# summa-dev/halo2-experiments

Measured on AMD Instinct MI355X. Metric: BN256 G1 MSM throughput, higher is better.
Workload: dtype u32; 1 GPU; standalone BN256 G1 MSM, 2^24 points per GPU (global 2^24 x 1; BASELINE configs[4] microbench, north-star headline size); points_per_gpu=16777216, global_points=16777216, base_set=fixed-base table (registration default from 2^17 points), window_bits=22, windows=12, parallelism=index-range shards x1, all-gather of 96 B partials (RCCL) + host fold, base_set_bytes=12901679104

## Files before the change

### halo2-experiments_amd/_lib.py

```python
from __future__ import annotations

import ctypes
import os
import subprocess

_HERE = os.path.dirname(os.path.abspath(__file__))
CSRC = os.path.join(_HERE, "csrc")
os.environ.setdefault("GPU_MAX_HW_QUEUES", "16")
LIB_PATH = os.environ.get("HALO2_MI355X_LIB") or os.path.join(CSRC, "libhalo2_mi355x.so")
HOSTCHECK_PATH = os.path.join(CSRC, "libhm_hostcheck.so")
HEADER_PATH = os.path.join(os.path.dirname(_HERE), "include", "halo2_mi355x.h")

_u64p = ctypes.POINTER(ctypes.c_uint64)
_vp = ctypes.c_void_p
NO_CHAIN = ctypes.c_size_t(-1).value


class Halo2Mi355xError(RuntimeError):
    def __init__(self, code: int, message: str):
        super().__init__(f"libhalo2_mi355x error {code}: {message}")
        self.code = code


class MsmStats(ctypes.Structure):
# ... 44 lines not shown
                                          ctypes.POINTER(ctypes.c_int)]),
    "hm_register_bases_dev": (ctypes.c_int, [_vp, ctypes.c_size_t, _vp, _u64p]),
    "hm_register_bases_precomp": (ctypes.c_int, [_u64p, ctypes.c_size_t, _u64p]),
    "hm_register_bases_precomp_dev": (ctypes.c_int, [_vp, ctypes.c_size_t, _vp, _u64p]),
    "hm_register_bases_plain": (ctypes.c_int, [_u64p, ctypes.c_size_t, _u64p]),
    "hm_register_bases_plain_dev": (ctypes.c_int, [_vp, ctypes.c_size_t, _vp, _u64p]),
    "hm_get_bases_info": (ctypes.c_int, [ctypes.c_uint64, ctypes.POINTER(BasesInfo)]),
    "hm_msm_bn256_g1_dev": (ctypes.c_int, [ctypes.c_uint64, ctypes.c_size_t, _vp, ctypes.c_size_t, _vp, _u64p]),
    "hm_msm_submit_dev": (ctypes.c_int, [ctypes.c_uint64, ctypes.c_size_t, _vp, ctypes.c_size_t, _vp, _u64p]),
    "hm_msm_wait": (ctypes.c_int, [ctypes.c_uint64, _u64p]),
    "hm_msm_batch_bn256_g1_dev": (ctypes.c_int, [ctypes.c_uint64, ctypes.c_size_t, ctypes.POINTER(ctypes.c_void_p), ctypes.c_size_t,
                                                 ctypes.c_size_t, _vp, _u64p]),
    "hm_msm_batch_bn256_g1_h": (ctypes.c_int, [ctypes.c_uint64, ctypes.c_size_t, ctypes.POINTER(ctypes.c_void_p), ctypes.c_size_t,
                                              ctypes.c_size_t, _u64p]),
    "hm_g1_sum": (ctypes.c_int, [_u64p, ctypes.c_size_t, _u64p]),
    "hm_coeff_to_extended_bn256_fr_dev": (ctypes.c_int, [ctypes.c_void_p, ctypes.c_void_p, ctypes.c_size_t, _u64p, ctypes.c_uint32,
                                                         ctypes.c_uint32, _u64p, ctypes.c_void_p]),
    "hm_coeff_to_coset_bn256_fr_dev": (ctypes.c_int, [_vp, _vp, ctypes.c_size_t, _u64p, ctypes.c_uint32, _u64p, ctypes.c_int, _vp]),
    "hm_coset_to_coeff_bn256_fr_dev": (ctypes.c_int, [_vp, ctypes.c_size_t, _u64p, ctypes.c_uint32, _u64p, _u64p, _vp]),
    "hm_coeff_to_cosets_bn256_fr_dev": (ctypes.c_int, [_vp, _vp, ctypes.c_size_t, _u64p, ctypes.c_uint32, _u64p, ctypes.c_size_t, ctypes.c_int, _vp]),
    "hm_cosets_to_coeff_bn256_fr_dev": (ctypes.c_int, [_vp, ctypes.c_size_t, _u64p, ctypes.c_uint32, _u64p, _u64p, _vp]),
    "hm_msm_set_window": (ctypes.c_int, [ctypes.c_int]),
    "hm_msm_set_phase_timing": (ctypes.c_int, [ctypes.c_int]),
    "hm_set_host_base_cache": (ctypes.c_int, [ctypes.c_int]),
    "hm_set_fixed_base_threshold": (ctypes.c_int, [ctypes.c_uint32]),
    "hm_set_msm_devices": (ctypes.c_int, [ctypes.POINTER(ctypes.c_int), ctypes.c_int]),
    "hm_ntt_bn256_fr": (ctypes.c_int, [_u64p, _u64p, ctypes.c_uint32]),
    "hm_set_host_copies": (ctypes.c_int, [ctypes.c_int]),
    "hm_host_register": (ctypes.c_int, [ctypes.c_void_p, ctypes.c_size_t]),
    "hm_host_unregister": (ctypes.c_int, [ctypes.c_void_p]),
# ... 100 lines not shown
```

### halo2-experiments_amd/csrc/capi.hip

```cpp
#include <hip/hip_runtime.h>

#include <cstdlib>

#include <atomic>
#include <chrono>
#include <string>
#include <map>
#include <random>
#include <stdexcept>
#include <thread>
#include <vector>

#include "hm_internal.h"
#include "host_fr.h"

namespace hm {

namespace {
struct HwQueueDefault {
  HwQueueDefault() { (void)setenv("GPU_MAX_HW_QUEUES", "16", 0); }
} g_hw_queue_default;
}

static thread_local std::string g_last_error;
// ... 33 lines not shown
long g_fault_after = -1;
void hm_fault_point(const char* point) {
  std::lock_guard<std::mutex> lk(g_fault_mu);
  if (g_fault_after < 0 || g_fault_name != point) return;
  if (g_fault_after-- == 0) throw std::runtime_error(std::string("injected fault at ") + point);
}
#endif

void msm_set_window_override(int c);
void msm_set_phase_timing(int mode);

static double now_us() {
  return std::chrono::duration<double, std::micro>(std::chrono::steady_clock::now().time_since_epoch()).count();
}

static void count_msm(DeviceCtx& ctx, size_t n, double device_ms) {
  uint32_t lg = 0;
  while ((n >> (lg + 1)) != 0) ++lg;
  ctx.calls.msm_calls += 1;
  ctx.calls.msm_points += n;
  ctx.calls.msm_by_log[lg & 31] += 1;
  ctx.calls.msm_device_us += device_ms * 1e3;
}

constexpr size_t kParkedBytesMax = (size_t)2 << 30;
static size_t parked_bytes(const DeviceCtx& ctx) {
  size_t t = 0;
  for (const auto& f : ctx.free_bases) t += f.xy_bytes + f.inf_bytes;
  return t;
}
static void free_bases_entry(DeviceCtx& ctx, BasesEntry& b) {
// ... 433 lines not shown
  if (!b) return hm_fail(HM_ERR_NOT_FOUND, "hm_get_bases_info: unknown handle");
  out->n = b->n;
  out->table_windows = b->pc_W;
  out->table_window_bits = b->pc_c;
  out->device_bytes = b->xy_bytes + b->inf_bytes;
  out->devices = 1;
  out->parked_bytes = parked_bytes(*ctx);
  return HM_OK;
} HM_API_CATCH("hm_get_bases_info")

int hm_release_bases(uint64_t handle) try {
  if (is_multi_handle(handle)) return multi_release(handle);
  DeviceCtx* ctx = ctx_for_current_device();
  if (!ctx) return HM_ERR_NO_DEVICE;
  std::lock_guard<std::mutex> lk(ctx->mu);
  for (size_t i = 0; i < ctx->bases.size(); ++i) {
    if (ctx->bases[i].handle == handle) {
      bool in_flight = false;
      for (int k = 1; k < HM_MSM_SLOTS; ++k)
        if (ctx->msm_slots[k].busy && ctx->msm_slots[k].bases_handle == handle) in_flight = true;
      if (in_flight) ctx->zombie_bases.push_back(ctx->bases[i]);
      else free_bases_entry(*ctx, ctx->bases[i]);
      ctx->bases.erase(ctx->bases.begin() + i);
      return HM_OK;
    }
  }
  return hm_fail(HM_ERR_NOT_FOUND, "hm_release_bases: unknown handle");
} HM_API_CATCH("hm_release_bases")

int hm_msm_bn256_g1_dev(uint64_t handle, size_t offset, const void* d_scalars, size_t n, void* stream, uint64_t out_xyz[12]) try {
// ... 3 lines not shown
    return multi_msm(handle, offset, d_scalars, false, n, stream, out_xyz, &id);
  }
  DeviceCtx* ctx = ctx_for_current_device();
  if (!ctx) return HM_ERR_NO_DEVICE;
  std::lock_guard<std::mutex> lk(ctx->mu);
  BasesEntry* b = find_bases(*ctx, handle);
  if (!b) return hm_fail(HM_ERR_NOT_FOUND, "hm_msm_bn256_g1_dev: unknown base handle");
  if (offset > b->n || n > b->n - offset) return hm_fail(HM_ERR_BAD_ARG, "hm_msm_bn256_g1_dev: offset + n exceeds the base set");
  int is_id = 0;
  const uint32_t pc = (offset == 0 && n == b->n) ? b->pc_c : 0u;
  const int rc = msm_run(*ctx, (const uint32_t*)d_scalars, b->d_xy + offset * 16, b->d_inf + offset, n, pc, out_xyz, &is_id,
                         (hipStream_t)stream);
  if (rc == HM_OK) count_msm(*ctx, n, ctx->last_msm.t_total_ms);
  return rc;
} HM_API_CATCH("hm_msm_bn256_g1_dev")

static int submit_chain(DeviceCtx* ctx, uint64_t handle, size_t offset, const void* const* d_scalars_list, uint32_t group, size_t n,
                        void* stream, uint64_t* out_ticket, const char* who, bool* all_busy = nullptr, bool use_table = true,
                        size_t live_rows = 0) {
  if (all_busy) *all_busy = false;
  std::lock_guard<std::mutex> lk(ctx->mu);
  BasesEntry* b = find_bases(*ctx, handle);
  if (!b) return hm_fail(HM_ERR_NOT_FOUND, std::string(who) + ": unknown base handle");
  if (offset > b->n || n > b->n - offset) return hm_fail(HM_ERR_BAD_ARG, std::string(who) + ": offset + n exceeds the base set");
  int slot = -1;
  for (int i = 1; i < HM_MSM_SLOTS; ++i)
    if (!ctx->msm_slots[i].busy) { slot = i; break; }
  if (slot < 0) {
    if (all_busy) *all_busy = true;
    return hm_fail(HM_ERR_BAD_ARG, std::string(who) + ": every slot is in flight; hm_msm_wait one first");
// ... 582 lines not shown

int hm_g1_sum(const uint64_t* points_xyz, size_t count, uint64_t out_xyz[12]) try {
  if (!out_xyz || (count && !points_xyz)) return hm_fail(HM_ERR_BAD_ARG, "hm_g1_sum: null argument");
  if (count > (1u << 20)) return hm_fail(HM_ERR_BAD_ARG, "hm_g1_sum: meant for a handful of partial results");
  hm_fault_point("g1_sum");
  int is_id = 0;
  host_sum_points(points_xyz, count, out_xyz, &is_id);
  return HM_OK;
} HM_API_CATCH("hm_g1_sum")

int hm_get_msm_stats(hm_msm_stats* out) try {
  if (!out) return hm_fail(HM_ERR_BAD_ARG, "hm_get_msm_stats: null output");
  DeviceCtx* ctx = ctx_for_current_device();
  if (!ctx) return HM_ERR_NO_DEVICE;
  std::lock_guard<std::mutex> lk(ctx->mu);
  const MsmStats& s = ctx->last_msm;
  out->digits_ms = s.t_digits_ms; out->sort_ms = s.t_sort_ms; out->accumulate_ms = s.t_accum_ms;
  out->reduce_ms = s.t_reduce_ms; out->total_ms = s.t_total_ms; out->accumulate_kernel_ms = s.t_accum_kernel_ms;
  out->pairs = s.pairs; out->tasks = s.tasks; out->window_bits = s.c; out->windows = s.windows;
  return HM_OK;
} HM_API_CATCH("hm_get_msm_stats")

int hm_get_stats(hm_stats* out) try {
  if (!out) return hm_fail(HM_ERR_BAD_ARG, "hm_get_stats: null output");
  DeviceCtx* ctx = ctx_for_current_device();
  if (!ctx) return HM_ERR_NO_DEVICE;
  std::lock_guard<std::mutex> lk(ctx->mu);
  const CallStats& c = ctx->calls;
  std::memset(out, 0, sizeof *out);
  out->msm_calls = c.msm_calls; out->msm_points = c.msm_points;
  out->ntt_calls = c.ntt_calls; out->ntt_elements = c.ntt_elements;
  for (int i = 0; i < 32; ++i) { out->msm_calls_by_log2[i] = c.msm_by_log[i]; out->ntt_calls_by_log2[i] = c.ntt_by_log[i]; }
  out->msm_h2d_us = c.msm_h2d_us; out->msm_device_us = c.msm_device_us; out->msm_host_us = c.msm_host_us;
  out->ntt_h2d_us = c.ntt_h2d_us; out->ntt_device_us = c.ntt_device_us; out->ntt_d2h_us = c.ntt_d2h_us;
  out->h2d_bytes = c.h2d_bytes; out->d2h_bytes = c.d2h_bytes;
  for (int i = 0; i < 8; ++i) { out->vector_calls[i] = c.vector_calls[i]; out->vector_elements[i] = c.vector_elements[i]; }
  out->coset_table_bytes = ctx->coset_table_bytes;
  out->coset_tables = ctx->coset_tables.size();
  out->ntt_table_bytes = ctx->ntt_table_bytes;
  out->ntt_tables = ctx->ntt_tables.size();
  out->host_copies_direct = ctx->xfer.direct.load(std::memory_order_relaxed);
  out->host_copies_staged = ctx->xfer.staged.load(std::memory_order_relaxed);
// ... 739 lines not shown
```

### halo2-experiments_amd/csrc/hm_internal.h

```cpp
#pragma once
#include <hip/hip_runtime.h>
#include <stdint.h>

#include <atomic>
#include <cstring>
#include <exception>
#include <functional>
#include <memory>
#include <mutex>
#include <string>
#include <thread>
#include <utility>
#include <vector>

#include "../../include/halo2_mi355x.h"

namespace hm {

int hm_fail(int code, const std::string& what);

#define HM_HIP_CHECK(expr)                                                                          \
  do {                                                                                              \
    hipError_t _e = (expr);                                                                         \
    if (_e != hipSuccess)                                                                           \
// ... 210 lines not shown
  std::vector<BasesEntry> zombie_bases;
  std::vector<FreeBases> free_bases;
  std::vector<std::unique_ptr<GraphProgram>> graphs;
  hipStream_t batch_streams[HM_MSM_SLOTS - 1] = {};
  hipEvent_t batch_event = nullptr;
  bool batch_streams_ready = false;
  DevBuf batch_io[HM_MSM_SLOTS - 1];
  DevBuf live_io;
  std::mutex live_mu;
  std::mutex batch_h_mu;
  uint64_t next_handle = 1;
  size_t cached_host_n = 0;
  const void* cached_xy = nullptr;
  uint64_t cached_digest[4] = {0, 0, 0, 0};
  MsmStats last_msm;
  CallStats calls;
  bool msm_attr_set = false, ntt_attr_set = false, msm_small_attr_set = false, lookup_attr_set = false;
};

AuxSlot* aux_acquire(DeviceCtx& ctx, hipStream_t stream);
int aux_release(DeviceCtx& ctx, AuxSlot* slot, hipStream_t stream);

DeviceCtx* ctx_for_current_device();

int xfer_h2d(DeviceCtx& ctx, void* d_dst, const void* src, size_t bytes, const char* who);
int xfer_d2h(DeviceCtx& ctx, void* dst, const void* d_src, size_t bytes, const char* who);
int xfer_many(DeviceCtx& ctx, bool up, void* const* dev, void* const* host, const size_t* bytes, size_t count, const char* who);
void xfer_release(DeviceCtx& ctx);
void xfer_prefault(void* p, size_t bytes);
int xfer_set_policy(int mode);
// ... 88 lines not shown
bool msm_phase_timing(bool small_plan);
int msm_slot_prepare(MsmSlot& sl);
int msm_launch_digits(const uint32_t* d_scalars_ext, const uint8_t* d_inf, int32_t* d_digits, size_t n, uint32_t c, uint32_t W,
                      hipStream_t stream);
bool msm_small_applies(size_t n, uint32_t c, bool single_set);
int msm_issue_small(DeviceCtx& ctx, int slot, const uint32_t* const* d_scalars_list, uint32_t group, const uint32_t* d_xy,
                    const uint8_t* d_inf, size_t n, uint32_t c, hipStream_t stream);
int msm_count_live_blocks(DeviceCtx& ctx, const void* const* d_columns, size_t count, const uint8_t* d_inf, size_t n, hipStream_t stream,
                          uint32_t* live_out);
bool msm_group_applies(size_t n, uint32_t precomp_c);
int msm_enqueue_group(DeviceCtx& ctx, int slot, const uint32_t* const* d_scalars_list, uint32_t group, const uint32_t* d_xy,
                      const uint8_t* d_inf, size_t n, hipStream_t stream, size_t live_rows = 0);
int msm_run(DeviceCtx& ctx, const uint32_t* d_scalars_ext, const uint32_t* d_xy, const uint8_t* d_inf, size_t n,
            uint32_t precomp_c, uint64_t out_jac_ext[12], int* out_is_identity, hipStream_t stream);
uint32_t msm_precomp_window(size_t n);
int msm_precompute(uint32_t* d_table, const uint8_t* d_inf, size_t n, uint32_t c, uint32_t W, hipStream_t stream);
void host_sum_points(const uint64_t* pts, size_t count, uint64_t out_jac_ext[12], int* out_is_identity);
int g1_fixed_base_mul_run(DeviceCtx& ctx, const uint32_t* d_scalars_ext, size_t n, const uint64_t base_affine_ext[8],
                          uint32_t* d_out_affine_ext, hipStream_t stream);

}
```

### halo2-experiments_amd/csrc/msm.hip

```cpp
#include <hip/hip_runtime.h>

#include <algorithm>
#include <chrono>
#include <cmath>
#include <cstdlib>

#include "hm_internal.h"
#include "host_fq.h"
#include "msm_dev.h"

namespace hm {


__global__ void msm_init_counters_kernel(uint32_t* __restrict__ bcnt, size_t nbt, uint32_t* __restrict__ br_count,
                                         uint32_t* __restrict__ khist, uint32_t nkeys, uint32_t* __restrict__ big_count) {
  const size_t i0 = (size_t)blockIdx.x * blockDim.x + threadIdx.x, stride = (size_t)gridDim.x * blockDim.x;
  for (size_t i = i0; i < nbt; i += stride) bcnt[i] = 0;
  if (i0 < nkeys) khist[i0] = 0;
  if (i0 < 4) {
    if (br_count) br_count[i0] = 0;
    big_count[i0] = 0;
  }
}

// ... 21 lines not shown

#ifndef HM_TARGET_TASKS
#define HM_TARGET_TASKS 327680
#endif
constexpr uint32_t TARGET_TASKS = HM_TARGET_TASKS;
__device__ __forceinline__ uint32_t effective_task_len(const uint32_t* __restrict__ pairs, uint32_t L_host) {
  if (pairs == nullptr) return L_host;
  const uint32_t by_fill = pairs[0] / TARGET_TASKS;
  const uint32_t L = L_host < by_fill ? L_host : by_fill;
  return L < 16u ? 16u : L;
}

struct MsmGroupScalars {
  const uint32_t* s[HM_MSM_GROUP];
};
__global__ void msm_digits_kernel(MsmGroupScalars list, const uint8_t* __restrict__ inf,
                                  int32_t* __restrict__ digits, size_t n, uint32_t c, uint32_t W, uint32_t n_wide) {
  const size_t i = (size_t)blockIdx.x * blockDim.x + threadIdx.x;
  if (i >= n) return;
  const uint32_t* __restrict__ scalars = list.s[blockIdx.y];
  digits += (size_t)blockIdx.y * W * n;
  const uint4* q = reinterpret_cast<const uint4*>(scalars + i * 8);
  const uint4 lo = q[0], hi = q[1];
  const uint32_t w_in[8] = {lo.x, lo.y, lo.z, lo.w, hi.x, hi.y, hi.z, hi.w};
  Fr k32 = fe_zero<FrParams>();
  k32.l[0] = 32;
  const Fr s = fe_canonical(fe_mul(fe_unpack<FrParams>(w_in), k32));
  uint32_t v[9];
  {
    uint32_t t[8];
    fe_pack(t, s);
#pragma unroll
    for (int k = 0; k < 8; ++k) v[k] = t[k];
    v[8] = 0;
  }
  const bool skip = inf[i] != 0;
  uint32_t carry = 0;
  for (uint32_t w = 0; w < W; ++w) {
    const uint32_t bits = w < n_wide ? c : c - 1;
    const uint32_t mask = (1u << bits) - 1u, half = 1u << (bits - 1);
    uint32_t d = (v[0] & mask) + carry;
    int32_t sd;
    if (d > half) {
      sd = (int32_t)d - (int32_t)(1u << bits);
      carry = 1;
    } else {
      sd = (int32_t)d;
      carry = 0;
    }
    digits[(size_t)w * n + i] = skip ? 0 : (w < n_wide ? sd : 2 * sd);
#pragma unroll
    for (int k = 0; k < 8; ++k) v[k] = __funnelshift_r(v[k], v[k + 1], bits);
  }
}

#ifndef HM_SORT_THREADS
#define HM_SORT_THREADS 1024
#endif
constexpr int SORT_THREADS = HM_SORT_THREADS;

template <class T, class F>
__device__ __forceinline__ void block_for_each_word(const T* __restrict__ base, size_t lo, size_t hi, F f) {
  size_t a = lo;
  while (a < hi && (reinterpret_cast<uintptr_t>(base + a) & (4 * sizeof(T) - 1))) ++a;
  const size_t nvec = (hi - a) / 4;
  if (threadIdx.x < a - lo) f(lo + threadIdx.x, base[lo + threadIdx.x]);
  const size_t tail = a + nvec * 4;
  if (threadIdx.x < hi - tail) f(tail + threadIdx.x, base[tail + threadIdx.x]);
// ... 12 lines not shown
__global__ __launch_bounds__(SORT_THREADS) void msm_part1_hist_kernel(const int32_t* __restrict__ digits,
                                                                      uint32_t* __restrict__ chist, size_t n, size_t chunk,
                                                                      uint32_t fb, uint32_t NC) {
  extern __shared__ uint32_t hist[];
  const uint32_t g = blockIdx.x, w = blockIdx.y, G = gridDim.x;
  for (uint32_t b = threadIdx.x; b < NC; b += SORT_THREADS) hist[b] = 0;
  __syncthreads();
  const size_t lo = (size_t)g * chunk, hi = lo + chunk < n ? lo + chunk : n;
  const int32_t* dw = digits + (size_t)w * n;
  block_for_each_word(dw, lo, hi, [&](size_t, int32_t d) {
    if (d != 0) (void)lds_inc(hist, ((uint32_t)(d < 0 ? -d : d) - 1u) >> fb);
  });
  __syncthreads();
  uint32_t* out = chist + ((size_t)w * G + g) * NC;
  for (uint32_t b = threadIdx.x; b < NC; b += SORT_THREADS) out[b] = hist[b];
}

__global__ __launch_bounds__(64) void msm_part1_scan_kernel(uint32_t* __restrict__ chist, uint32_t* __restrict__ ctot, uint32_t G,
                                                            uint32_t NC, uint32_t W) {
  const uint32_t idx = blockIdx.x;
  if (idx >= W * NC) return;
  const uint32_t w = idx / NC, b = idx - w * NC;
  const uint32_t lane = threadIdx.x;
  const uint32_t per = (G + 63) / 64;
  const uint32_t lo = lane * per, hi = lo + per < G ? lo + per : G;
  uint32_t sum = 0;
  for (uint32_t g = lo; g < hi; ++g) sum += chist[((size_t)w * G + g) * NC + b];
  uint32_t incl = sum;
#pragma unroll
  for (int off = 1; off < 64; off <<= 1) {
// ... 1429 lines not shown
  return v;
}

struct BigRegionPlan {
  uint32_t big = 0;
  uint32_t slice = 0;
  uint32_t capacity = 0;
  uint2* list = nullptr;
  uint32_t* count = nullptr;
  uint32_t* gcursor = nullptr;
};

template <class ITEM>
static int launch_sort(const int32_t* d_digits, uint32_t* d_chist, uint32_t* d_ctot, uint32_t* d_cstart, void* d_tmp,
                       uint32_t* d_bcnt, size_t sn, size_t chunk, uint32_t G, uint32_t SW, uint32_t fb, uint32_t ib, uint32_t cb,
                       uint32_t NC, uint32_t NBP, const BigRegionPlan& br, hipStream_t stream) {
  const size_t lds_fine = (size_t)4 << fb;
  if (cb) {
    const size_t lds_coarse = (size_t)NC * 4;
    hipLaunchKernelGGL(msm_part1_hist_kernel, dim3(G, SW), dim3(SORT_THREADS), lds_coarse, stream, d_digits, d_chist, sn, chunk,
                       fb, NC);
    hipLaunchKernelGGL(msm_part1_scan_kernel, dim3(SW * NC), dim3(64), 0, stream, d_chist, d_ctot, G, NC, SW);
    hipLaunchKernelGGL(msm_part1_starts_kernel, dim3(1), dim3(1024), 0, stream, (const uint32_t*)d_ctot, d_cstart, SW * NC);
    static const bool big_tiles = [] { const char* v = std::getenv("HALO2_MI355X_P1_BIG_TILES"); return !(v && *v == '0'); }();
    static const uint32_t p1_big_from = [] { const char* v = std::getenv("HALO2_MI355X_P1_BIG_FROM"); return (uint32_t)(v && *v ? std::atoi(v) : 512); }();
    if (sizeof(ITEM) == 4 && NC <= 4096 && !sort_v1()) {
      if (NC >= (p1_big_from) && NC <= 2048 && big_tiles) {
        constexpr int TILE = SORT_THREADS * P1_BIG_IPT;
        hipLaunchKernelGGL((msm_part1_scatter_v2_kernel<P1_BIG_IPT>), dim3(G, SW), dim3(SORT_THREADS), ((size_t)3 * NC + 32 + 2 * TILE) * 4, stream,
                           d_digits, (const uint32_t*)d_chist, (const uint32_t*)d_cstart, (uint32_t*)d_tmp, sn, chunk, fb, ib, NC);
      } else {
        constexpr int TILE = SORT_THREADS * P1_IPT_DEFAULT;
        hipLaunchKernelGGL((msm_part1_scatter_v2_kernel<P1_IPT_DEFAULT>), dim3(G, SW), dim3(SORT_THREADS), ((size_t)3 * NC + 32 + 2 * TILE) * 4,
                           stream, d_digits, (const uint32_t*)d_chist, (const uint32_t*)d_cstart, (uint32_t*)d_tmp, sn, chunk, fb, ib, NC);
      }
    } else if (NC >= (p1_big_from) && NC <= 2048 && sizeof(ITEM) == 4 && big_tiles) {
// ... 301 lines not shown
  sl.res_stride = res_stride;
  sl.live_ptr = nullptr;
  sl.phase_timed = msm_phase_timing(false);
  const bool pt = sl.phase_timed;
  sl.T_max = T_max;
  sl.d_win = d_win;
  sl.d_tot = d_tot;
  HM_HIP_CHECK(hipEventRecord(ev[0], stream));

  uint32_t n_wide = W;
  if (single_set) {
    uint32_t wide;
    balanced_windows(W, &wide, &n_wide);
    if (wide != c) return hm_fail(HM_ERR_INTERNAL, "msm: the base set's table was built for another window split");
  }
  {
    MsmGroupScalars list;
    for (uint32_t e = 0; e < (uint32_t)HM_MSM_GROUP; ++e) list.s[e] = d_scalars_list[e < group ? e : 0];
    hipLaunchKernelGGL(msm_digits_kernel, dim3((uint32_t)((n + 255) / 256), group), dim3(256), 0, stream, list, d_inf, d_digits, n, c, W,
                       n_wide);
  }
  HM_HIP_CHECK(hipGetLastError());
  if (pt) HM_HIP_CHECK(hipEventRecord(ev[1], stream));

  {
    {
      const uint32_t blocks = (uint32_t)std::min<size_t>(((size_t)NBT + 255) / 256, 2048);
      hipLaunchKernelGGL(msm_init_counters_kernel, dim3(blocks < 4 ? 4 : blocks), dim3(256), 0, stream, d_bcnt, (size_t)NBT,
                         cb ? br.count : (uint32_t*)nullptr, d_khist, TASK_KEYS, d_big_count);
      HM_HIP_CHECK(hipGetLastError());
    }
    const int rc = wide_items
                       ? launch_sort<uint64_t>(d_digits, d_chist, d_ctot, d_cstart, d_tmp, d_bcnt, sn, chunk, G, SW, fb, ib, cb,
                                               NC, NBP, br, stream)
                       : launch_sort<uint32_t>(d_digits, d_chist, d_ctot, d_cstart, d_tmp, d_bcnt, sn, chunk, G, SW, fb, ib, cb,
                                               NC, NBP, br, stream);
    if (rc != HM_OK) return rc;
  }
  const uint32_t* d_pairs = cb ? (const uint32_t*)(d_cstart + (size_t)SW * NC) : (const uint32_t*)nullptr;
  {
    const uint32_t nblocks = (NBT + SCAN_BLOCK - 1) / SCAN_BLOCK;
    hipLaunchKernelGGL(msm_scan_partial_kernel, dim3(nblocks), dim3(SCAN_THREADS), 0, stream, (const uint32_t*)d_bcnt,
                       d_bsum, NBT, d_pairs, L);
    hipLaunchKernelGGL(msm_scan_blocksums_kernel, dim3(1), dim3(SCAN_THREADS), 0, stream, d_bsum, nblocks, d_tot,
                       (uint32_t)std::min<uint64_t>(T_max, 0xffffffffull));
    hipLaunchKernelGGL(msm_scan_final_kernel, dim3(nblocks), dim3(SCAN_THREADS), 0, stream, (const uint32_t*)d_bcnt,
                       (const uint32_t*)d_bsum, d_boff, d_toff, (const uint32_t*)d_tot, NBT, d_pairs, L,
                       coop_sort ? br.gcursor : (uint32_t*)nullptr);
    HM_HIP_CHECK(hipGetLastError());
  }
  {
// ... 172 lines not shown
  ctx.last_msm.c = sl.c;
  ctx.last_msm.windows = sl.W;
}

int msm_finish(DeviceCtx& ctx, int slot, uint64_t out_jac_ext[12], int* out_is_identity) {
  double host_us = 0;
  const int rc = msm_finish_wait_fold(ctx.msm_slots[slot], out_jac_ext, out_is_identity, &host_us);
  if (rc == HM_OK) msm_finish_record(ctx, slot, host_us);
  else ctx.msm_slots[slot].live_ptr = nullptr;
  return rc;
}

int msm_run(DeviceCtx& ctx, const uint32_t* d_scalars_ext, const uint32_t* d_xy, const uint8_t* d_inf, size_t n,
            uint32_t precomp_c, uint64_t out_jac_ext[12], int* out_is_identity, hipStream_t stream) {
  if (ctx.msm_slots[0].busy) return hm_fail(HM_ERR_BAD_ARG, "msm: slot 0 is held by an un-awaited hm_msm_submit_dev ticket");
  const int rc = msm_enqueue(ctx, 0, d_scalars_ext, d_xy, d_inf, n, precomp_c, stream);
  if (rc != HM_OK) return rc;
  return msm_finish(ctx, 0, out_jac_ext, out_is_identity);
}

int g1_fixed_base_mul_run(DeviceCtx& ctx, const uint32_t* d_scalars_ext, size_t n, const uint64_t base_affine_ext[8],
                          uint32_t* d_out_affine_ext, hipStream_t stream) {
  if (n == 0) return HM_OK;
  AuxSlot* slot = aux_acquire(ctx, stream);
  if (!slot) return HM_ERR_HIP;
  uint32_t* d_table = (uint32_t*)slot->table.ensure((size_t)64 * 15 * PT_WORDS * 4);
  if (!d_table) return hm_fail(HM_ERR_HIP, "fixed-base: table allocation failed");
  G1AffineWords base;
  std::memcpy(base.w, base_affine_ext, 64);
  hipLaunchKernelGGL(g1_fixed_table_kernel, dim3(1), dim3(64), 0, stream, base, d_table);
  HM_HIP_CHECK(hipGetLastError());
  hipLaunchKernelGGL(g1_fixed_base_mul_kernel, dim3((uint32_t)((n + ACC_THREADS - 1) / ACC_THREADS)), dim3(ACC_THREADS), 0,
                     stream, d_scalars_ext, (const uint32_t*)d_table, d_out_affine_ext, n);
// ... 6 lines not shown
```

### halo2-experiments_amd/sharding.py

```python
from __future__ import annotations

import ctypes
import os
from typing import Callable, Optional, Tuple

import numpy as np

from . import _lib
from .arithmetic import _ptr, best_multiexp


def shard_range(n: int, rank: int, world: int) -> Tuple[int, int]:
    if not (0 <= rank < world):
        raise ValueError("rank out of range")
    q, r = divmod(n, world)
    lo = rank * q + min(rank, r)
    return lo, lo + q + (1 if rank < r else 0)


def g1_sum(points: np.ndarray) -> np.ndarray:
    pts = np.ascontiguousarray(points, dtype=np.uint64).reshape(-1, 12)
    out = np.zeros(12, dtype=np.uint64)
    _lib.check(_lib.load().hm_g1_sum(_ptr(pts), pts.shape[0], _ptr(out)))
    return out
# ... 11 lines not shown
    return bool(force_collective)


def _comm_device(group):
    import torch
    import torch.distributed as dist

    return torch.device("cuda", torch.cuda.current_device()) if dist.get_backend(group) == "nccl" else torch.device("cpu")


def sharded_multiexp(local_coeffs, local_bases, group=None,
                     local_msm: Optional[Callable] = None, force_collective: Optional[bool] = None) -> np.ndarray:
    import torch
    import torch.distributed as dist

    partial = (local_msm or best_multiexp)(local_coeffs, local_bases)
    if not _exchanges(group, force_collective):
        return g1_sum(partial.reshape(1, 12))
    world = dist.get_world_size(group)
    dev = _comm_device(group)
    mine = torch.from_numpy(partial.view(np.int64).copy()).to(dev)
    gathered = [torch.empty_like(mine) for _ in range(world)]
    dist.all_gather(gathered, mine, group=group)
    pts = torch.stack(gathered).cpu().numpy().view(np.uint64)
    return g1_sum(pts)


MAX_IN_FLIGHT = 8
_NO_GROUP = object()


def sharded_multiexp_batch(jobs, group=None, streams=None, local_batch: Optional[Callable] = None,
                           force_collective: Optional[bool] = None) -> np.ndarray:
    import torch
    import torch.distributed as dist

    if local_batch is not None:
        partials = np.stack([np.asarray(p, dtype=np.uint64).reshape(12) for p in local_batch(jobs)]) if jobs else np.zeros((0, 12), np.uint64)
    else:
        partials = np.zeros((len(jobs), 12), dtype=np.uint64)
# ... 92 lines not shown
```

### include/halo2_mi355x.h

```cpp
#ifndef HALO2_MI355X_H
#define HALO2_MI355X_H

#include <stddef.h>
#include <stdint.h>

#ifdef __cplusplus
extern "C" {
#endif

#define HM_OK 0
#define HM_ERR_BAD_ARG (-1)
#define HM_ERR_NO_DEVICE (-2)
#define HM_ERR_HIP (-3)
#define HM_ERR_NOT_FOUND (-4)
#define HM_ERR_INTERNAL (-5)
#define HM_ERR_PARTIAL_OUTPUT (-6)


int hm_set_device(int device);
int hm_device_count(void);
int hm_shutdown(void);
const char* hm_last_error(void);
const char* hm_version(void);

// ... 16 lines not shown
typedef struct hm_bases_info {
  uint64_t n;
  uint64_t device_bytes;
  uint64_t parked_bytes;
  uint64_t default_tables_dropped;
  uint32_t table_windows;
  uint32_t table_window_bits;
  uint32_t devices;
  uint32_t sliced;
} hm_bases_info;
int hm_get_bases_info(uint64_t handle, hm_bases_info* out);

int hm_register_bases_dev(const void* d_bases, size_t n, void* stream, uint64_t* out_handle);
int hm_msm_bn256_g1_dev(uint64_t handle, size_t offset, const void* d_scalars, size_t n, void* stream,
                        uint64_t out_xyz[12]);

int hm_msm_submit_dev(uint64_t handle, size_t offset, const void* d_scalars, size_t n, void* stream, uint64_t* out_ticket);
int hm_msm_wait(uint64_t ticket, uint64_t out_xyz[12]);
int hm_msm_batch_bn256_g1_dev(uint64_t handle, size_t offset, const void* const* d_scalars, size_t n, size_t count, void* stream,
                              uint64_t* out_xyz);
int hm_msm_batch_bn256_g1_h(uint64_t handle, size_t offset, const uint64_t* const* scalars, size_t n, size_t count, uint64_t* out_xyz);

int hm_set_msm_devices(const int* devices, int count);

int hm_g1_sum(const uint64_t* points_xyz, size_t count, uint64_t out_xyz[12]);

int hm_set_host_base_cache(int enable);

int hm_device_malloc(size_t bytes, void** d_out);
int hm_device_free(void* d_ptr);
// ... 136 lines not shown
```

### rust/halo2-mi355x-sys/src/lib.rs

```rust
#![allow(non_camel_case_types)]

use std::ffi::CStr;
use std::os::raw::{c_char, c_int, c_long, c_void};

pub const HM_OK: c_int = 0;
pub const HM_ERR_BAD_ARG: c_int = -1;
pub const HM_ERR_NO_DEVICE: c_int = -2;
pub const HM_ERR_HIP: c_int = -3;
pub const HM_ERR_NOT_FOUND: c_int = -4;
pub const HM_ERR_INTERNAL: c_int = -5;
pub const HM_ERR_PARTIAL_OUTPUT: c_int = -6;
pub const HM_GRAPH_COLUMNS_INTERNAL: c_int = 1;
pub const HM_STAT_EVAL_POLYNOMIAL: c_int = 0;
pub const HM_STAT_GRAPH_EVALUATE: c_int = 1;
pub const HM_STAT_KATE_DIVISION: c_int = 2;
pub const HM_STAT_GRAND_PRODUCT: c_int = 3;
pub const HM_STAT_BATCH_INVERT: c_int = 4;
pub const HM_STAT_LINEAR_COMBINATION: c_int = 5;
pub const HM_STAT_LOOKUP_PERMUTE: c_int = 6;

#[repr(C)]
#[derive(Clone, Copy, Debug)]
pub struct HmBasesInfo {
    pub n: u64,
    pub device_bytes: u64,
    pub parked_bytes: u64,
// ... 54 lines not shown
    pub fn hm_last_error() -> *const c_char;
    pub fn hm_version() -> *const c_char;
    pub fn hm_msm_bn256_g1(scalars: *const u64, bases: *const u64, n: usize, out_xy: *mut u64, out_is_identity: *mut c_int) -> c_int;
    pub fn hm_msm_bn256_g1_jacobian(scalars: *const u64, bases: *const u64, n: usize, out_xyz: *mut u64) -> c_int;
    pub fn hm_register_bases(bases: *const u64, n: usize, out_handle: *mut u64) -> c_int;
    pub fn hm_release_bases(handle: u64) -> c_int;
    pub fn hm_msm_bn256_g1_h(handle: u64, offset: usize, scalars: *const u64, n: usize, out_xy: *mut u64, out_is_identity: *mut c_int) -> c_int;
    pub fn hm_register_bases_precomp(bases: *const u64, n: usize, out_handle: *mut u64) -> c_int;
    pub fn hm_register_bases_precomp_dev(d_bases: *const c_void, n: usize, stream: *mut c_void, out_handle: *mut u64) -> c_int;
    pub fn hm_set_fixed_base_threshold(log2_n: u32) -> c_int;
    pub fn hm_register_bases_plain(bases: *const u64, n: usize, out_handle: *mut u64) -> c_int;
    pub fn hm_register_bases_plain_dev(d_bases: *const c_void, n: usize, stream: *mut c_void, out_handle: *mut u64) -> c_int;
    pub fn hm_get_bases_info(handle: u64, out: *mut HmBasesInfo) -> c_int;
    pub fn hm_register_bases_dev(d_bases: *const c_void, n: usize, stream: *mut c_void, out_handle: *mut u64) -> c_int;
    pub fn hm_msm_bn256_g1_dev(handle: u64, offset: usize, d_scalars: *const c_void, n: usize, stream: *mut c_void, out_xyz: *mut u64) -> c_int;
    pub fn hm_msm_submit_dev(handle: u64, offset: usize, d_scalars: *const c_void, n: usize, stream: *mut c_void, out_ticket: *mut u64) -> c_int;
    pub fn hm_msm_wait(ticket: u64, out_xyz: *mut u64) -> c_int;
    pub fn hm_msm_batch_bn256_g1_dev(handle: u64, offset: usize, d_scalars: *const *const c_void, n: usize, count: usize,
        stream: *mut c_void, out_xyz: *mut u64) -> c_int;
    pub fn hm_msm_batch_bn256_g1_h(handle: u64, offset: usize, scalars: *const *const u64, n: usize, count: usize, out_xyz: *mut u64) -> c_int;
    pub fn hm_set_msm_devices(devices: *const c_int, count: c_int) -> c_int;
    pub fn hm_g1_sum(points_xyz: *const u64, count: usize, out_xyz: *mut u64) -> c_int;
    pub fn hm_set_host_base_cache(enable: c_int) -> c_int;
    pub fn hm_device_malloc(bytes: usize, d_out: *mut *mut c_void) -> c_int;
    pub fn hm_device_free(d_ptr: *mut c_void) -> c_int;
    pub fn hm_copy_to_device(d_dst: *mut c_void, src: *const c_void, bytes: usize) -> c_int;
    pub fn hm_copy_to_host(dst: *mut c_void, d_src: *const c_void, bytes: usize) -> c_int;
    pub fn hm_copy_many_to_device(d_dsts: *const *mut c_void, srcs: *const *const c_void, bytes: *const usize, count: usize) -> c_int;
    pub fn hm_copy_many_to_host(dsts: *const *mut c_void, d_srcs: *const *const c_void, bytes: *const usize, count: usize) -> c_int;
    pub fn hm_device_synchronize() -> c_int;
// ... 77 lines not shown
```

Before: 948.4 million points/s.

## Fuse digit extraction with coarse histogram and export raw records for sharded MSM

Adds a fused kernel that computes signed window digits and builds the per-chunk coarse histogram in LDS in one pass, so the separate histogram kernel and its re-read of the digits array are skipped when the chunking fits. It also adds a records path for sharded MSM: each rank exports its raw window landing data to a device buffer, all-gathers that block, and folds every rank's windows on the host. This avoids the host sync and per-rank host fold before the collective. The cost is a larger all-gather payload, deferred bookkeeping through a settle step, and per-point LDS atomics in the digits kernel.

```diff
diff --git a/halo2-experiments_amd/_lib.py b/halo2-experiments_amd/_lib.py
--- a/halo2-experiments_amd/_lib.py
+++ b/halo2-experiments_amd/_lib.py
@@ -82,6 +82,8 @@
     "hm_msm_batch_bn256_g1_h": (ctypes.c_int, [ctypes.c_uint64, ctypes.c_size_t, ctypes.POINTER(ctypes.c_void_p), ctypes.c_size_t,
                                               ctypes.c_size_t, _u64p]),
     "hm_g1_sum": (ctypes.c_int, [_u64p, ctypes.c_size_t, _u64p]),
+    "hm_msm_bn256_g1_dev_records": (ctypes.c_int, [ctypes.c_uint64, ctypes.c_size_t, _vp, ctypes.c_size_t, _vp, _vp]),
+    "hm_msm_fold_records": (ctypes.c_int, [_vp, ctypes.c_size_t, _u64p]),
     "hm_coeff_to_extended_bn256_fr_dev": (ctypes.c_int, [ctypes.c_void_p, ctypes.c_void_p, ctypes.c_size_t, _u64p, ctypes.c_uint32,
                                                          ctypes.c_uint32, _u64p, ctypes.c_void_p]),
     "hm_coeff_to_coset_bn256_fr_dev": (ctypes.c_int, [_vp, _vp, ctypes.c_size_t, _u64p, ctypes.c_uint32, _u64p, ctypes.c_int, _vp]),
diff --git a/halo2-experiments_amd/csrc/capi.hip b/halo2-experiments_amd/csrc/capi.hip
--- a/halo2-experiments_amd/csrc/capi.hip
+++ b/halo2-experiments_amd/csrc/capi.hip
@@ -71,7 +71,7 @@
   return std::chrono::duration<double, std::micro>(std::chrono::steady_clock::now().time_since_epoch()).count();
 }
 
-static void count_msm(DeviceCtx& ctx, size_t n, double device_ms) {
+void count_msm(DeviceCtx& ctx, size_t n, double device_ms) {
   uint32_t lg = 0;
   while ((n >> (lg + 1)) != 0) ++lg;
   ctx.calls.msm_calls += 1;
@@ -535,6 +535,10 @@
   DeviceCtx* ctx = ctx_for_current_device();
   if (!ctx) return HM_ERR_NO_DEVICE;
   std::lock_guard<std::mutex> lk(ctx->mu);
+  {
+    const int rs = msm_settle_records(*ctx);
+    if (rs != HM_OK) return rs;
+  }
   for (size_t i = 0; i < ctx->bases.size(); ++i) {
     if (ctx->bases[i].handle == handle) {
       bool in_flight = false;
@@ -568,6 +572,36 @@
   if (rc == HM_OK) count_msm(*ctx, n, ctx->last_msm.t_total_ms);
   return rc;
 } HM_API_CATCH("hm_msm_bn256_g1_dev")
+
+int hm_msm_bn256_g1_dev_records(uint64_t handle, size_t offset, const void* d_scalars, size_t n, void* stream, void* d_records) try {
+  if (!d_records || (n && !d_scalars)) return hm_fail(HM_ERR_BAD_ARG, "hm_msm_bn256_g1_dev_records: null argument");
+  if (is_multi_handle(handle)) return hm_fail(HM_ERR_BAD_ARG, "hm_msm_bn256_g1_dev_records: a multi-device handle folds its own parts");
+  DeviceCtx* ctx = ctx_for_current_device();
+  if (!ctx) return HM_ERR_NO_DEVICE;
+  std::lock_guard<std::mutex> lk(ctx->mu);
+  BasesEntry* b = find_bases(*ctx, handle);
+  if (!b) return hm_fail(HM_ERR_NOT_FOUND, "hm_msm_bn256_g1_dev_records: unknown base handle");
+  if (offset > b->n || n > b->n - offset) return hm_fail(HM_ERR_BAD_ARG, "hm_msm_bn256_g1_dev_records: offset + n exceeds the base set");
+  int rc = msm_settle_records(*ctx);
+  if (rc != HM_OK) return rc;
+  if (ctx->msm_slots[0].busy) return hm_fail(HM_ERR_BAD_ARG, "msm: slot 0 is held by an un-awaited hm_msm_submit_dev ticket");
+  const uint32_t pc = (offset == 0 && n == b->n) ? b->pc_c : 0u;
+  rc = msm_enqueue(*ctx, 0, (const uint32_t*)d_scalars, b->d_xy + offset * 16, b->d_inf + offset, n, pc, (hipStream_t)stream);
+  if (rc == HM_OK) rc = msm_export_records(*ctx, 0, d_records);
+  if (rc != HM_OK) {
+    ctx->msm_slots[0].live_ptr = nullptr;
+    return rc;
+  }
+  ctx->msm_records_pending = n != 0;
+  return HM_OK;
+} HM_API_CATCH("hm_msm_bn256_g1_dev_records")
+
+int hm_msm_fold_records(const void* records, size_t count, uint64_t out_xyz[12]) try {
+  if (!out_xyz || (count && !records)) return hm_fail(HM_ERR_BAD_ARG, "hm_msm_fold_records: null argument");
+  if (count > 4096) return hm_fail(HM_ERR_BAD_ARG, "hm_msm_fold_records: meant for one block per rank");
+  int is_id = 0;
+  return msm_fold_records((const uint32_t*)records, count, out_xyz, &is_id);
+} HM_API_CATCH("hm_msm_fold_records")
 
 static int submit_chain(DeviceCtx* ctx, uint64_t handle, size_t offset, const void* const* d_scalars_list, uint32_t group, size_t n,
                         void* stream, uint64_t* out_ticket, const char* who, bool* all_busy = nullptr, bool use_table = true,
@@ -1180,6 +1214,10 @@
   DeviceCtx* ctx = ctx_for_current_device();
   if (!ctx) return HM_ERR_NO_DEVICE;
   std::lock_guard<std::mutex> lk(ctx->mu);
+  {
+    const int rs = msm_settle_records(*ctx);
+    if (rs != HM_OK) return rs;
+  }
   const MsmStats& s = ctx->last_msm;
   out->digits_ms = s.t_digits_ms; out->sort_ms = s.t_sort_ms; out->accumulate_ms = s.t_accum_ms;
   out->reduce_ms = s.t_reduce_ms; out->total_ms = s.t_total_ms; out->accumulate_kernel_ms = s.t_accum_kernel_ms;
@@ -1192,6 +1230,10 @@
   DeviceCtx* ctx = ctx_for_current_device();
   if (!ctx) return HM_ERR_NO_DEVICE;
   std::lock_guard<std::mutex> lk(ctx->mu);
+  {
+    const int rs = msm_settle_records(*ctx);
+    if (rs != HM_OK) return rs;
+  }
   const CallStats& c = ctx->calls;
   std::memset(out, 0, sizeof *out);
   out->msm_calls = c.msm_calls; out->msm_points = c.msm_points;
diff --git a/halo2-experiments_amd/csrc/hm_internal.h b/halo2-experiments_amd/csrc/hm_internal.h
--- a/halo2-experiments_amd/csrc/hm_internal.h
+++ b/halo2-experiments_amd/csrc/hm_internal.h
@@ -248,6 +248,7 @@
   const void* cached_xy = nullptr;
   uint64_t cached_digest[4] = {0, 0, 0, 0};
   MsmStats last_msm;
+  bool msm_records_pending = false;
   CallStats calls;
   bool msm_attr_set = false, ntt_attr_set = false, msm_small_attr_set = false, lookup_attr_set = false;
 };
@@ -366,6 +367,10 @@
 int msm_run(DeviceCtx& ctx, const uint32_t* d_scalars_ext, const uint32_t* d_xy, const uint8_t* d_inf, size_t n,
             uint32_t precomp_c, uint64_t out_jac_ext[12], int* out_is_identity, hipStream_t stream);
 uint32_t msm_precomp_window(size_t n);
+int msm_export_records(DeviceCtx& ctx, int slot, void* d_out);
+int msm_fold_records(const uint32_t* blocks, size_t count, uint64_t out_jac_ext[12], int* out_is_identity);
+int msm_settle_records(DeviceCtx& ctx);
+void count_msm(DeviceCtx& ctx, size_t n, double device_ms);
 int msm_precompute(uint32_t* d_table, const uint8_t* d_inf, size_t n, uint32_t c, uint32_t W, hipStream_t stream);
 void host_sum_points(const uint64_t* pts, size_t count, uint64_t out_jac_ext[12], int* out_is_identity);
 int g1_fixed_base_mul_run(DeviceCtx& ctx, const uint32_t* d_scalars_ext, size_t n, const uint64_t base_affine_ext[8],
diff --git a/halo2-experiments_amd/csrc/msm.hip b/halo2-experiments_amd/csrc/msm.hip
--- a/halo2-experiments_amd/csrc/msm.hip
+++ b/halo2-experiments_amd/csrc/msm.hip
@@ -59,14 +59,8 @@
 struct MsmGroupScalars {
   const uint32_t* s[HM_MSM_GROUP];
 };
-__global__ void msm_digits_kernel(MsmGroupScalars list, const uint8_t* __restrict__ inf,
-                                  int32_t* __restrict__ digits, size_t n, uint32_t c, uint32_t W, uint32_t n_wide) {
-  const size_t i = (size_t)blockIdx.x * blockDim.x + threadIdx.x;
-  if (i >= n) return;
-  const uint32_t* __restrict__ scalars = list.s[blockIdx.y];
-  digits += (size_t)blockIdx.y * W * n;
-  const uint4* q = reinterpret_cast<const uint4*>(scalars + i * 8);
-  const uint4 lo = q[0], hi = q[1];
+template <class F>
+__device__ __forceinline__ void point_digits(const uint4 lo, const uint4 hi, bool skip, uint32_t c, uint32_t W, uint32_t n_wide, F emit) {
   const uint32_t w_in[8] = {lo.x, lo.y, lo.z, lo.w, hi.x, hi.y, hi.z, hi.w};
   Fr k32 = fe_zero<FrParams>();
   k32.l[0] = 32;
@@ -79,7 +73,6 @@
     for (int k = 0; k < 8; ++k) v[k] = t[k];
     v[8] = 0;
   }
-  const bool skip = inf[i] != 0;
   uint32_t carry = 0;
   for (uint32_t w = 0; w < W; ++w) {
     const uint32_t bits = w < n_wide ? c : c - 1;
@@ -93,10 +86,20 @@
       sd = (int32_t)d;
       carry = 0;
     }
-    digits[(size_t)w * n + i] = skip ? 0 : (w < n_wide ? sd : 2 * sd);
+    emit(w, skip ? 0 : (w < n_wide ? sd : 2 * sd));
 #pragma unroll
     for (int k = 0; k < 8; ++k) v[k] = __funnelshift_r(v[k], v[k + 1], bits);
   }
+}
+
+__global__ void msm_digits_kernel(MsmGroupScalars list, const uint8_t* __restrict__ inf,
+                                  int32_t* __restrict__ digits, size_t n, uint32_t c, uint32_t W, uint32_t n_wide) {
+  const size_t i = (size_t)blockIdx.x * blockDim.x + threadIdx.x;
+  if (i >= n) return;
+  const uint32_t* __restrict__ scalars = list.s[blockIdx.y];
+  digits += (size_t)blockIdx.y * W * n;
+  const uint4* q = reinterpret_cast<const uint4*>(scalars + i * 8);
+  point_digits(q[0], q[1], inf[i] != 0, c, W, n_wide, [&](uint32_t w, int32_t d) { digits[(size_t)w * n + i] = d; });
 }
 
 #ifndef HM_SORT_THREADS
@@ -139,6 +142,53 @@
   __syncthreads();
   uint32_t* out = chist + ((size_t)w * G + g) * NC;
   for (uint32_t b = threadIdx.x; b < NC; b += SORT_THREADS) out[b] = hist[b];
+}
+
+constexpr size_t DIGITS_HIST_LDS_MAX = 64 * 1024;
+constexpr int DIGITS_AHEAD = 4;
+__global__ __launch_bounds__(SORT_THREADS) void msm_digits_hist_kernel(MsmGroupScalars list, const uint8_t* __restrict__ inf,
+                                                                       int32_t* __restrict__ digits, uint32_t* __restrict__ chist,
+                                                                       size_t n, size_t chunk, uint32_t c, uint32_t W,
+                                                                       uint32_t n_wide, uint32_t fb, uint32_t NC) {
+  extern __shared__ uint32_t hist[];
+  const uint32_t g = blockIdx.x, e = blockIdx.y, GP = gridDim.x, tid = threadIdx.x;
+  const uint32_t WNC = W * NC;
+  for (uint32_t b = tid; b < WNC; b += SORT_THREADS) hist[b] = 0;
+  __syncthreads();
+  const uint32_t* __restrict__ scalars = list.s[e];
+  digits += (size_t)e * W * n;
+  const size_t lo = (size_t)g * chunk, hi = lo + chunk < n ? lo + chunk : n;
+  constexpr int D = DIGITS_AHEAD;
+  uint4 a0[D], a1[D];
+  uint8_t f[D];
+  auto fetch = [&](int k, size_t p) {
+    if (p < hi) {
+      const uint4* q = reinterpret_cast<const uint4*>(scalars + p * 8);
+      a0[k] = q[0];
+      a1[k] = q[1];
+      f[k] = inf[p];
+    }
+  };
+#pragma unroll
+  for (int k = 0; k < D; ++k) fetch(k, lo + tid + (size_t)k * SORT_THREADS);
+  for (size_t i = lo + tid; i < hi; i += (size_t)D * SORT_THREADS) {
+#pragma unroll
+    for (int k = 0; k < D; ++k) {
+      const size_t p = i + (size_t)k * SORT_THREADS;
+      if (p < hi) {
+        point_digits(a0[k], a1[k], f[k] != 0, c, W, n_wide, [&](uint32_t w, int32_t d) {
+          digits[(size_t)w * n + p] = d;
+          if (d != 0) (void)lds_inc(hist + w * NC, ((uint32_t)(d < 0 ? -d : d) - 1u) >> fb);
+        });
+      }
+      fetch(k, p + (size_t)D * SORT_THREADS);
+    }
+  }
+  __syncthreads();
+  for (uint32_t b = tid; b < WNC; b += SORT_THREADS) {
+    const uint32_t w = b / NC;
+    chist[(((size_t)e * W + w) * GP + g) * NC + (b - w * NC)] = hist[b];
+  }
 }
 
 __global__ __launch_bounds__(64) void msm_part1_scan_kernel(uint32_t* __restrict__ chist, uint32_t* __restrict__ ctot, uint32_t G,
@@ -1598,12 +1648,13 @@
 template <class ITEM>
 static int launch_sort(const int32_t* d_digits, uint32_t* d_chist, uint32_t* d_ctot, uint32_t* d_cstart, void* d_tmp,
                        uint32_t* d_bcnt, size_t sn, size_t chunk, uint32_t G, uint32_t SW, uint32_t fb, uint32_t ib, uint32_t cb,
-                       uint32_t NC, uint32_t NBP, const BigRegionPlan& br, hipStream_t stream) {
+                       uint32_t NC, uint32_t NBP, const BigRegionPlan& br, bool chist_done, hipStream_t stream) {
   const size_t lds_fine = (size_t)4 << fb;
   if (cb) {
     const size_t lds_coarse = (size_t)NC * 4;
-    hipLaunchKernelGGL(msm_part1_hist_kernel, dim3(G, SW), dim3(SORT_THREADS), lds_coarse, stream, d_digits, d_chist, sn, chunk,
-                       fb, NC);
+    if (!chist_done)
+      hipLaunchKernelGGL(msm_part1_hist_kernel, dim3(G, SW), dim3(SORT_THREADS), lds_coarse, stream, d_digits, d_chist, sn, chunk,
+                         fb, NC);
     hipLaunchKernelGGL(msm_part1_scan_kernel, dim3(SW * NC), dim3(64), 0, stream, d_chist, d_ctot, G, NC, SW);
     hipLaunchKernelGGL(msm_part1_starts_kernel, dim3(1), dim3(1024), 0, stream, (const uint32_t*)d_ctot, d_cstart, SW * NC);
     static const bool big_tiles = [] { const char* v = std::getenv("HALO2_MI355X_P1_BIG_TILES"); return !(v && *v == '0'); }();
@@ -1935,11 +1986,16 @@
     balanced_windows(W, &wide, &n_wide);
     if (wide != c) return hm_fail(HM_ERR_INTERNAL, "msm: the base set's table was built for another window split");
   }
+  const bool chist_in_k0 = cb != 0 && n % chunk == 0 && (size_t)G * chunk == sn && (size_t)W * NC * 4 <= DIGITS_HIST_LDS_MAX;
   {
     MsmGroupScalars list;
     for (uint32_t e = 0; e < (uint32_t)HM_MSM_GROUP; ++e) list.s[e] = d_scalars_list[e < group ? e : 0];
-    hipLaunchKernelGGL(msm_digits_kernel, dim3((uint32_t)((n + 255) / 256), group), dim3(256), 0, stream, list, d_inf, d_digits, n, c, W,
-                       n_wide);
+    if (chist_in_k0)
+      hipLaunchKernelGGL(msm_digits_hist_kernel, dim3((uint32_t)(n / chunk), group), dim3(SORT_THREADS), (size_t)W * NC * 4, stream, list,
+                         d_inf, d_digits, d_chist, n, chunk, c, W, n_wide, fb, NC);
+    else
+      hipLaunchKernelGGL(msm_digits_kernel, dim3((uint32_t)((n + 255) / 256), group), dim3(256), 0, stream, list, d_inf, d_digits, n, c,
+                         W, n_wide);
   }
   HM_HIP_CHECK(hipGetLastError());
   if (pt) HM_HIP_CHECK(hipEventRecord(ev[1], stream));
@@ -1953,9 +2009,9 @@
     }
     const int rc = wide_items
                        ? launch_sort<uint64_t>(d_digits, d_chist, d_ctot, d_cstart, d_tmp, d_bcnt, sn, chunk, G, SW, fb, ib, cb,
-                                               NC, NBP, br, stream)
+                                               NC, NBP, br, chist_in_k0, stream)
                        : launch_sort<uint32_t>(d_digits, d_chist, d_ctot, d_cstart, d_tmp, d_bcnt, sn, chunk, G, SW, fb, ib, cb,
-                                               NC, NBP, br, stream);
+                                               NC, NBP, br, chist_in_k0, stream);
     if (rc != HM_OK) return rc;
   }
   const uint32_t* d_pairs = cb ? (const uint32_t*)(d_cstart + (size_t)SW * NC) : (const uint32_t*)nullptr;
@@ -2158,9 +2214,75 @@
 int msm_run(DeviceCtx& ctx, const uint32_t* d_scalars_ext, const uint32_t* d_xy, const uint8_t* d_inf, size_t n,
             uint32_t precomp_c, uint64_t out_jac_ext[12], int* out_is_identity, hipStream_t stream) {
   if (ctx.msm_slots[0].busy) return hm_fail(HM_ERR_BAD_ARG, "msm: slot 0 is held by an un-awaited hm_msm_submit_dev ticket");
+  const int rs = msm_settle_records(ctx);
+  if (rs != HM_OK) return rs;
   const int rc = msm_enqueue(ctx, 0, d_scalars_ext, d_xy, d_inf, n, precomp_c, stream);
   if (rc != HM_OK) return rc;
   return msm_finish(ctx, 0, out_jac_ext, out_is_identity);
+}
+
+constexpr uint32_t REC_MAGIC = 0x31524d48u;
+constexpr uint32_t REC_HDR_WORDS = 40;
+static_assert(HM_MSM_RECORDS_BYTES == (REC_HDR_WORDS + 4 + 128 * 32) * 4, "record block size");
+struct MsmRecordHeader {
+  uint32_t w[REC_HDR_WORDS];
+};
+__global__ void msm_export_records_kernel(MsmRecordHeader hdr, const uint32_t* __restrict__ src, uint32_t words,
+                                          uint32_t* __restrict__ dst) {
+  if (threadIdx.x == 0) {
+#pragma unroll
+    for (uint32_t k = 0; k < REC_HDR_WORDS; ++k) dst[k] = hdr.w[k];
+  }
+  for (uint32_t i = threadIdx.x; i < words; i += blockDim.x) dst[REC_HDR_WORDS + i] = src[i];
+}
+
+int msm_export_records(DeviceCtx& ctx, int slot, void* d_out) {
+  MsmSlot& sl = ctx.msm_slots[slot];
+  MsmRecordHeader hdr{};
+  hdr.w[0] = REC_MAGIC;
+  uint32_t words = 0;
+  if (sl.n != 0) {
+    if (sl.group != 1 || sl.SW > 128) return hm_fail(HM_ERR_INTERNAL, "msm: a record block holds one MSM of <= 128 windows");
+    words = 4 + sl.SW * 32;
+    hdr.w[1] = sl.SW;
+    hdr.w[2] = sl.c;
+    hdr.w[3] = sl.balanced ? 1u : 0u;
+    hdr.w[4] = words;
+    if (sl.balanced) std::memcpy(&hdr.w[8], sl.win_bits, 128);
+  }
+  uint32_t* d_land = nullptr;
+  if (words) HM_HIP_CHECK(hipHostGetDevicePointer((void**)&d_land, sl.h_land, 0));
+  hipLaunchKernelGGL(msm_export_records_kernel, dim3(1), dim3(256), 0, sl.stream, hdr, (const uint32_t*)d_land, words, (uint32_t*)d_out);
+  HM_HIP_CHECK(hipGetLastError());
+  if (words) HM_HIP_CHECK(hipEventRecord(sl.ev[4], sl.stream));
+  return HM_OK;
+}
+
+int msm_settle_records(DeviceCtx& ctx) {
+  if (!ctx.msm_records_pending) return HM_OK;
+  ctx.msm_records_pending = false;
+  MsmSlot& sl = ctx.msm_slots[0];
+  HM_HIP_CHECK(hipEventSynchronize(sl.ev[4]));
+  msm_finish_record(ctx, 0, 0.0);
+  count_msm(ctx, sl.n, ctx.last_msm.t_total_ms);
+  return HM_OK;
+}
+
+int msm_fold_records(const uint32_t* blocks, size_t count, uint64_t out_jac_ext[12], int* out_is_identity) {
+  std::vector<uint64_t> parts(count * 12, 0);
+  for (size_t r = 0; r < count; ++r) {
+    const uint32_t* b = blocks + r * (HM_MSM_RECORDS_BYTES / 4);
+    const uint32_t SW = b[1], words = b[4];
+    if (b[0] != REC_MAGIC || SW > 128 || (SW == 0 ? words != 0 : words != 4 + SW * 32))
+      return hm_fail(HM_ERR_BAD_ARG, "hm_msm_fold_records: not a record block of hm_msm_bn256_g1_dev_records");
+    if (SW == 0) continue;
+    const uint32_t* land = b + REC_HDR_WORDS;
+    if (land[2] != 0) return hm_fail(HM_ERR_INTERNAL, "msm: task count exceeds its bound");
+    int is_id = 0;
+    host_fold(land + 4, SW, b[2], &parts[r * 12], &is_id, b[3] ? reinterpret_cast<const uint8_t*>(&b[8]) : nullptr);
+  }
+  host_sum_points(parts.data(), count, out_jac_ext, out_is_identity);
+  return HM_OK;
 }
 
 int g1_fixed_base_mul_run(DeviceCtx& ctx, const uint32_t* d_scalars_ext, size_t n, const uint64_t base_affine_ext[8],
diff --git a/halo2-experiments_amd/sharding.py b/halo2-experiments_amd/sharding.py
--- a/halo2-experiments_amd/sharding.py
+++ b/halo2-experiments_amd/sharding.py
@@ -49,8 +49,11 @@
     import torch
     import torch.distributed as dist
 
+    exchange = _exchanges(group, force_collective)
+    if exchange and local_msm is None and _records_route(local_coeffs, local_bases, group):
+        return _sharded_multiexp_records(local_coeffs, local_bases, group)
     partial = (local_msm or best_multiexp)(local_coeffs, local_bases)
-    if not _exchanges(group, force_collective):
+    if not exchange:
         return g1_sum(partial.reshape(1, 12))
     world = dist.get_world_size(group)
     dev = _comm_device(group)
@@ -59,6 +62,48 @@
     dist.all_gather(gathered, mine, group=group)
     pts = torch.stack(gathered).cpu().numpy().view(np.uint64)
     return g1_sum(pts)
+
+
+RECORDS_BYTES = 16560
+
+
+def _records_route(local_coeffs, local_bases, group) -> bool:
+    from .arithmetic import BasesHandle, _is_tensor, bases_info
+
+    if not (isinstance(local_bases, BasesHandle) and _is_tensor(local_coeffs) and local_coeffs.device == _comm_device(group)):
+        return False
+    single = getattr(local_bases, "_single_device", None)
+    if single is None:
+        single = local_bases._single_device = bases_info(local_bases)["devices"] == 1
+    return single
+
+
+def _sharded_multiexp_records(local_coeffs, local_bases, group) -> np.ndarray:
+    import torch
+    import torch.distributed as dist
+
+    from .arithmetic import _stream_ptr, _tensor_rows
+
+    world = dist.get_world_size(group)
+    dev = local_coeffs.device
+    n = _tensor_rows(local_coeffs, 4, "coeffs")
+    cache = _RECORD_BUFFERS.get((dev, world))
+    if cache is None:
+        flat = torch.empty(world * RECORDS_BYTES, dtype=torch.uint8, device=dev)
+        cache = _RECORD_BUFFERS[(dev, world)] = (torch.empty(RECORDS_BYTES, dtype=torch.uint8, device=dev), flat,
+                                                 [flat[r * RECORDS_BYTES:(r + 1) * RECORDS_BYTES] for r in range(world)])
+    mine, gathered, views = cache
+    lib = _lib.load()
+    _lib.check(lib.hm_msm_bn256_g1_dev_records(ctypes.c_uint64(local_bases.handle), 0, ctypes.c_void_p(local_coeffs.data_ptr()), n,
+                                               ctypes.c_void_p(_stream_ptr(local_coeffs)), ctypes.c_void_p(mine.data_ptr())))
+    dist.all_gather(views, mine, group=group)
+    host = gathered.cpu().numpy()
+    out = np.zeros(12, dtype=np.uint64)
+    _lib.check(lib.hm_msm_fold_records(ctypes.c_void_p(host.ctypes.data), world, _ptr(out)))
+    return out
+
+
+_RECORD_BUFFERS: dict = {}
 
 
 MAX_IN_FLIGHT = 8
diff --git a/include/halo2_mi355x.h b/include/halo2_mi355x.h
--- a/include/halo2_mi355x.h
+++ b/include/halo2_mi355x.h
@@ -54,6 +54,11 @@
 int hm_register_bases_dev(const void* d_bases, size_t n, void* stream, uint64_t* out_handle);
 int hm_msm_bn256_g1_dev(uint64_t handle, size_t offset, const void* d_scalars, size_t n, void* stream,
                         uint64_t out_xyz[12]);
+
+#define HM_MSM_RECORDS_BYTES 16560
+int hm_msm_bn256_g1_dev_records(uint64_t handle, size_t offset, const void* d_scalars, size_t n, void* stream,
+                                void* d_records);
+int hm_msm_fold_records(const void* records, size_t count, uint64_t out_xyz[12]);
 
 int hm_msm_submit_dev(uint64_t handle, size_t offset, const void* d_scalars, size_t n, void* stream, uint64_t* out_ticket);
 int hm_msm_wait(uint64_t ticket, uint64_t out_xyz[12]);
diff --git a/rust/halo2-mi355x-sys/src/lib.rs b/rust/halo2-mi355x-sys/src/lib.rs
--- a/rust/halo2-mi355x-sys/src/lib.rs
+++ b/rust/halo2-mi355x-sys/src/lib.rs
@@ -10,6 +10,7 @@
 pub const HM_ERR_NOT_FOUND: c_int = -4;
 pub const HM_ERR_INTERNAL: c_int = -5;
 pub const HM_ERR_PARTIAL_OUTPUT: c_int = -6;
+pub const HM_MSM_RECORDS_BYTES: c_int = 16560;
 pub const HM_GRAPH_COLUMNS_INTERNAL: c_int = 1;
 pub const HM_STAT_EVAL_POLYNOMIAL: c_int = 0;
 pub const HM_STAT_GRAPH_EVALUATE: c_int = 1;
@@ -94,6 +95,9 @@
     pub fn hm_get_bases_info(handle: u64, out: *mut HmBasesInfo) -> c_int;
     pub fn hm_register_bases_dev(d_bases: *const c_void, n: usize, stream: *mut c_void, out_handle: *mut u64) -> c_int;
     pub fn hm_msm_bn256_g1_dev(handle: u64, offset: usize, d_scalars: *const c_void, n: usize, stream: *mut c_void, out_xyz: *mut u64) -> c_int;
+    pub fn hm_msm_bn256_g1_dev_records(handle: u64, offset: usize, d_scalars: *const c_void, n: usize, stream: *mut c_void,
+        d_records: *mut c_void) -> c_int;
+    pub fn hm_msm_fold_records(records: *const c_void, count: usize, out_xyz: *mut u64) -> c_int;
     pub fn hm_msm_submit_dev(handle: u64, offset: usize, d_scalars: *const c_void, n: usize, stream: *mut c_void, out_ticket: *mut u64) -> c_int;
     pub fn hm_msm_wait(ticket: u64, out_xyz: *mut u64) -> c_int;
     pub fn hm_msm_batch_bn256_g1_dev(handle: u64, offset: usize, d_scalars: *const *const c_void, n: usize, count: usize,
```

Result: no change. 952.5 million points/s (median of 6 runs) (+0.4%).
